# LinjianMa/pairwise-perturbation

Hardware: AMD Instinct MI355X
Metric: ALS sweeps/sec (exact dimension-tree sweep, CP order-4 s=200 R=10) (higher is better)
Workload: dtype f32

## Files before the change

pairwise-perturbation_amd/csrc/engine.cpp:

```cpp
#include "engine.h"
#include "assignment.h"
#include "run_report.h"

#include <algorithm>
#include <cmath>
#include <cstdio>
#include <cstdlib>
#include <cstring>
#include <fstream>
#include <iostream>
#include <limits>
#include <stdexcept>

namespace ppals {

int tensor_create(Ops &ops, Comm &comm, int order, const int64_t *glens, int dtype,
                  TensorDesc *out, std::string *err) {
  if (order < 2 || order > MAX_ORDER) {
    *err = "tensor order must be in [2, 8]";
    return -1;
  }
  if (!ops.supports_storage(dtype))
    throw Unsupported(dtype == BF16 ? "ppals: this back end cannot store a bf16 tensor"
                                    : "ppals: this back end cannot store this tensor type");
// ... 817 lines not shown
    ops_.zero(gradW_[i], n);
    maxs_ = std::max(maxs_, V_.glens[i]);
    maxblk_ = std::max(maxblk_, block_rows(V_.glens[i], P_));
  }
  const size_t sys_n = multi_ ? (size_t)tab_.sq[K_] : (size_t)R_ * R_;
  G_ = DeviceBuffer(ops_, sizeof(double) * N_ * sys_n);
  S_ = DeviceBuffer(ops_, sizeof(double) * sys_n);
  Sinv_ = DeviceBuffer(ops_, sizeof(double) * sys_n);
  gradsq_ = DeviceBuffer(ops_, sizeof(double) * MAX_ORDER * K_);
  scal_ = DeviceBuffer(ops_, sizeof(double) * 4 * MAX_ORDER);
  ops_.zero(gradsq_.as<double>(), sizeof(double) * MAX_ORDER * K_);
  if (dist_) {
    size_t n = sizeof(double) * (size_t)maxblk_ * P_ * R_;
    sendbuf_ = DeviceBuffer(ops_, n);
    recvbuf_ = DeviceBuffer(ops_, sizeof(double) * (size_t)maxblk_ * R_);
    gatherbuf_ = DeviceBuffer(ops_, n);
    ops_.zero(sendbuf_.as<double>(), n);
    ops_.zero(gatherbuf_.as<double>(), n);
  }
  if (const char *e = std::getenv("PPALS_COMM_SMALL_BYTES")) small_msg_bytes_ = std::atoll(e);
  if (const char *e = std::getenv("PPALS_TEST_BLOCKED_UPDATE")) test_blocks_ = std::atoi(e);
  if (N_ < 3) schedule_ = 0;
  if (const char *e = std::getenv("PPALS_PLACE_TUNE")) ms_tune_enabled_ = std::atoi(e) != 0;
  if (const char *e = std::getenv("PPALS_PACK_LAYOUT")) pack_mode_ = std::atoi(e) >= 0 && std::atoi(e) <= 2 ? std::atoi(e) : -1;
  if (N_ >= 3) {
    ms_set_roots(ms_choose_roots());
    ms_scales_ = DeviceBuffer(ops_, sizeof(double) * 32);
  }
  if (V_.generation) tensor_gen_ = *V_.generation;
  {
    Layout nat;
    nat.ptr = V_.data;
    for (int m = 0; m < N_; m++) nat.order.push_back(m);
    lay_.push_back(std::move(nat));
  }
  size_t xmax = 0;
  const bool place = schedule_ == 1 && N_ >= 3 && ms_tune_enabled_ && ms_X_slack() > 0;
  if (place) {
    for (int r = 0; r < N_; r++) {
      if (ms_set_excluded(r, ms_k_, ms_excl_)) continue;
      xmax = std::max(xmax, ms_X_bytes(r, ms_k_));
    }
    const size_t avail = ops_.mem_available();
    const double tensor_bytes = (double)V_.nloc * dtype_size(V_.dtype);
    if (avail == (size_t)-1 || (double)avail > 2.0 * tensor_bytes + 6.0 * (double)(xmax + ms_X_slack()) + 8e9)
      ms_X_alt_ = DeviceBuffer::try_alloc(ops_, xmax + ms_X_slack());
// ... 1134 lines not shown
    ms_start_step(r);
    return;
  }
  const void *src = pl.lay->ptr;
  const int64_t L = pl.Lc, J = pl.J, T = pl.T;
  ms_X_.modes = pl.kept;
  std::vector<FactorRef> f;
  unsigned mask = 0;
  for (int m : pl.set) {
    f.push_back(fref(m, W_.data()));
    mask |= 1u << m;
  }
  ms_X_.dt = work_dt(V_.dtype);
  ms_X_.contracted = mask;
  if ((size_t)L * T * R_ * dtype_size(ms_X_.dt) != xbytes)
    throw std::runtime_error("ppals: internal error (first-level intermediate size)");
  PackedSrc pk_store;
  const PackedSrc *pk = pl.Lc > 1 ? packed_for(pl, pk_store) : nullptr;
  auto launch_scan = [&](int blk, int64_t off, int nt) {
    ms_X_.buf = ms_X_override_ ? (char *)ms_X_override_
                               : (blk == 1 && ms_X_alt_ ? ms_X_alt_ : ms_X_base_).as<char>() + off;
    ops_.scan_store_mode(nt);
    PackedScope scope(ops_, pk);
    ops_.scan_contract(src, V_.dtype, pl.L, J, T, f.data(), (int)f.size(), R_, ms_X_.buf, ms_X_.dt,
                       L, L * T, pl.pad);
    ops_.scan_store_mode(-1);
  };
  PlaceExplore &ex = ms_place_[first];
  if (slack > 0 && !ms_X_override_ && ex.phase < 0) {
    static const int64_t cand_small[] = {0, 1, 2, 3, 4, 5, 6, 8, 12, 16, 24, 32, 48, 64};
    static const int64_t cand_large[] = {0, 3, 5, 12, 16, 24, 48, 64};
    const double bytes = (double)L * J * T * dtype_size(V_.dtype);
    ex.phase = 3;
    ex.layout = (int)(pl.lay - lay_.data());
    if (bytes >= place_min_bytes() && R_ <= 32 && (double)xbytes >= 0.01 * bytes) {
      const bool large = bytes >= 2e10;
      const int64_t *mb = large ? cand_large : cand_small;
      for (int ci = 0; ci < (large ? 8 : 14); ci++) {
        if ((size_t)(mb[ci] << 20) > slack) break;
        PlaceCand c;
        c.off = mb[ci] << 20;
        ex.cands.push_back(c);
      }
      static const int64_t cand_alt[] = {0, 4, 16, 64};
      for (int ci = 0; ms_X_alt_ && ci < 4; ci++) {
        if ((size_t)(cand_alt[ci] << 20) > slack) break;
        PlaceCand c;
        c.blk = 1;
        c.off = cand_alt[ci] << 20;
        ex.cands.push_back(c);
      }
      ex.phase = 0;
    }
  }
  const int cand = (slack > 0 && !ms_X_override_ && ex.phase >= 0 && ex.phase < 2) ? ms_place_pick(ex) : -1;
  if (cand >= 0) {
    ex.visits++;
    ex.timer_cand = cand;
    ex.timer = ops_.timer_begin();
    launch_scan(ex.cands[cand].blk, ex.cands[cand].off, ex.cands[cand].nt);
    if (ex.timer >= 0) ops_.timer_end(ex.timer);
  } else if (ex.phase == 2 && ex.chosen >= 0 && slack > 0 && !ms_X_override_) {
    launch_scan(ex.cands[ex.chosen].blk, ex.cands[ex.chosen].off, ex.cands[ex.chosen].nt);
  } else {
    launch_scan(0, 0, -1);
  }
  ms_X_.pending = false;
  ms_X_.valid = true;
  if (const char *tr = std::getenv("PPALS_TRACE_STEPS")) {
    if (FILE *f = std::fopen(tr, "a")) {
      const int li = (int)(pl.lay - lay_.data());
      std::fprintf(f, "rank=%d root=%d k=%d layout=%s%s L=%lld J=%lld T=%lld\n", rank_, first, k,
                   li == 1 ? "VT" : "V", pl.lay->q > 0 ? "pad" : "", (long long)L, (long long)J,
                   (long long)T);
      std::fclose(f);
    }
  }
}

void CpEngine::ms_mode_update(int i, double lambda, bool last_of_sweep) {
  check_tensor_generation();
  if (kind_[i] == kModeFixed) return;
  if (ms_root_ < 0 || ((i - ms_root_ + N_) % N_) < ms_k_) {
    const int first = ms_next_root(i, ms_k_, ms_excl_);
    if (first < 0) throw std::runtime_error("ppals: no root set without the excluded modes");
    ms_start_step(first);
  }
  int pos = -1;
  for (size_t q = 0; q < ms_order_.size(); q++)
    if (ms_order_[q] == i) pos = (int)q;
  const int leaf = ms_leaf_[pos];
  const bool free_i = kind_[i] == kModeFree;
  if (!multi_ && free_i) ops_.arm_gram_system(G_.as<double>(), N_, i, R_, lambda, S_.as<double>(), Sinv_.as<double>());
  ms_compute(leaf);
  ms_norm_fused_ = false;
  if (last_of_sweep && !multi_ && free_i && !skips_normalize() && (!dist_ || (i != 0 && (int64_t)sizeof(double) * V_.glens[i] * R_ <= small_msg_bytes_))) {
    int64_t rows[MAX_ORDER];
    for (int q = 0; q < N_; q++) rows[q] = V_.glens[q];
    if (ops_.arm_normalize(W_.data(), rows, N_, R_, G_.as<double>(), i, nullptr)) {
      unsigned masks[32] = {0}, fresh = 0;
      const unsigned active = ms_collect_scales(masks, &fresh, leaf);
      ms_norm_fused_ = ops_.arm_normalize(W_.data(), rows, N_, R_, G_.as<double>(), i, nullptr,
                                          ms_scales_.as<double>(), masks, active, fresh);
    }
  }
  mode_update(i, (const double *)ms_nodes_[leaf].t.buf, ext(i), lambda, false, 1.0);
  ms_nodes_[leaf].t.valid = false;
  for (auto &nd : ms_nodes_)
    if (nd.t.contracted & (1u << i)) nd.t.valid = false;
}

void CpEngine::ms_contract(const RTensor &src, int mode, RTensor &dst, DeviceBuffer &own, const double *in_scale) {
  int64_t L = 1, T = 1;
  bool before = true;
  dst.modes.clear();
  for (int m : src.modes) {
    if (m == mode) {
      before = false;
      continue;
    }
    (before ? L : T) *= ext(m);
    dst.modes.push_back(m);
  }
  dst.dt = F64;
  dst.contracted = src.contracted | (1u << mode);
  own.reserve(ops_, sizeof(double) * (size_t)L * T * R_);
  dst.buf = own.get();
  FactorRef f = fref(mode, W_.data());
// ... 15 lines not shown
  auto storage_pos = [&](int mode) {
    for (size_t k = 0; k < src->modes.size(); k++)
      if (src->modes[k] == mode) return (int)k;
    return -1;
  };
  std::sort(sib.begin(), sib.end(), [&](int a, int b) { return storage_pos(a) > storage_pos(b); });
  if (n.tmp.size() + 1 < sib.size()) {
    n.tmp.resize(sib.size() - 1);
    n.tmp_own.resize(sib.size() - 1);
  }
  const RTensor *cur = src;
  for (size_t k = 0; k < sib.size(); k++) {
    const bool last = k + 1 == sib.size();
    RTensor &dst = last ? n.t : n.tmp[k];
    ms_contract(*cur, sib[k], dst, last ? n.own : n.tmp_own[k], k == 0 ? ms_scale_of(*src) : nullptr);
    cur = &dst;
  }
  if (sib.empty()) throw std::runtime_error("ppals: empty sibling set in the multi-sweep tree");
  n.t.pending = false;
  n.t.valid = true;
}

void CpEngine::sweep_msdt(double lambda) {
  for (int i = 0; i < N_; i++) ms_mode_update(i, lambda, i == N_ - 1);
  if (!ms_norm_fused_ && !skips_normalize()) normalize();
  ms_norm_fused_ = false;
  grad_from_sweep_ = true;
}

void CpEngine::sweep_dt(double lambda) {
  if (schedule_ == 1) {
    sweep_msdt(lambda);
    return;
  }
  for (auto &n : nodes_) n.valid = false;
  bool norm_fused = false;
  for (int i = 0; i < N_; i++) {
    if (kind_[i] == kModeFixed) continue;
    compute_node(leaf_[i]);
    const Node &lf = nodes_[leaf_[i]];
    if (i == N_ - 1 && !dist_ && kind_[i] == kModeFree && !skips_normalize()) {
      int64_t rows[MAX_ORDER];
      for (int q = 0; q < N_; q++) rows[q] = V_.glens[q];
      norm_fused = ops_.arm_normalize(W_.data(), rows, N_, R_, G_.as<double>(), i, nullptr);
    }
    mode_update(i, lf.buf.as<double>(), ext(i), lambda, false, 1.0);
  }
// ... 1470 lines not shown
```

pairwise-perturbation_amd/csrc/engine.h:

```cpp
#pragma once
#include <cstdint>
#include <cstdlib>
#include <functional>
#include <map>
#include <string>
#include <vector>

#include "device_buffer.h"
#include "ops.h"

namespace ppals {

struct TensorDesc {
  int order = 0;
  int64_t glens[MAX_ORDER];
  int64_t llens[MAX_ORDER];
  int64_t row0 = 0;
  int dtype = F32;
  void *data = nullptr;
  int64_t nloc = 0;
  uint64_t *generation = nullptr;
  uint64_t *prep_epoch = nullptr;
};

// ... 252 lines not shown
    std::vector<RTensor> tmp;
    DeviceBuffer own;
    std::vector<DeviceBuffer> tmp_own;
  };
  void ms_build_tree(int lo, int hi, int parent);
  void ms_start_step(int root);
  void ms_compute(int idx);
  void ms_contract(const RTensor &src, int mode, RTensor &dst, DeviceBuffer &own, const double *in_scale);
  void sweep_msdt(double lambda);
  void ms_invalidate() { ms_root_ = -1; }
  int schedule_ = 1;
  int ms_root_ = -1;
  int ms_k_ = 1;
  int test_blocks_ = 0;
  DeviceBuffer test_blkbuf_;
  unsigned ms_excl_ = 0;
  bool ms_set_excluded(int first, int k, unsigned excl) const;
  int ms_next_root(int i, int k, unsigned excl) const;
  double ms_schedule_cost(int k, unsigned excl) const;
  int ms_choose_roots();
  void ms_set_roots(int k);
  void ms_mode_update(int i, double lambda, bool last_of_sweep = false);
  bool ms_norm_fused_ = false;
  unsigned ms_collect_scales(unsigned *masks, unsigned *fresh, int skip_node);
  RTensor ms_X_;
  struct PlaceCand {
    int blk = 0;
    int64_t off = 0;
    int nt = -1;
    double best = 1e300;
    int samples = 0;
  };
  struct PlaceExplore {
    int phase = -1;
    size_t next = 0;
    int timer = -1;
    int timer_cand = -1;
    int chosen = -1;
    int layout = 0;
    double worst = 0;
    int visits = 0;
    bool gated = false;
    std::vector<PlaceCand> cands;
  };
  static constexpr int kPlaceGateSamples = 8;
  static constexpr double kPlaceGateSpread = 0.04;
// ... 163 lines not shown
```

pairwise-perturbation_amd/csrc/hip_ops.hip:

```cpp
#include <dlfcn.h>
#include <hip/hip_runtime.h>
#include <chrono>

#include <algorithm>
#include <cstdio>
#include <cstdlib>
#include <stdexcept>
#include <string>
#include <map>
#include <type_traits>
#include <vector>

#include "hip_ops.h"
#include "roctx_ranges.h"
#include "preload_policy.h"
#include "kernels_scan.hip.h"
#include "kernels_pack.hip.h"
#include "kernels_small.hip.h"
#include "kernels_nn.hip.h"
#include "kernels_polar.hip.h"
#include "kernels_shape.hip.h"
#include "kernels_holdout.hip.h"
#include "kernels_corcondia.hip.h"
#include "kernels_fms.hip.h"
// ... 187 lines not shown
    HIP_CHECK(hipFuncSetAttribute((const void *)k_polar_factor, hipFuncAttributeMaxDynamicSharedMemorySize,
                                  96 * 1024));
    HIP_CHECK(hipFuncSetAttribute((const void *)k_shape_columns, hipFuncAttributeMaxDynamicSharedMemorySize,
                                  (int)kShapeLdsBytes));
    HIP_CHECK(hipFuncSetAttribute((const void *)k_p2_polar, hipFuncAttributeMaxDynamicSharedMemorySize, 96 * 1024));
    const void *p2_wide[] = {(const void *)k_p2_project<float, 4>, (const void *)k_p2_project<double, 4>};
    for (const void *k : p2_wide)
      HIP_CHECK(hipFuncSetAttribute(k, hipFuncAttributeMaxDynamicSharedMemorySize, (int)p2_project_lds(64)));
  }
  ~HipOps() override {
    hipSetDevice(dev_);
    hipStreamSynchronize(st_);
    if (st2_) hipStreamSynchronize(st2_);
    for (auto &ev : events_) {
      hipEventDestroy(ev.a);
      hipEventDestroy(ev.b);
    }
    for (auto &t : timers_) {
      hipEventDestroy(t.a);
      hipEventDestroy(t.b);
    }
    if (ws_mttv_) hipFree(ws_mttv_);
    if (ws_pack_) hipFree(ws_pack_);
    if (pack_stats_) hipFree(pack_stats_);
    if (ws_mv_) hipFree(ws_mv_);
    if (ws_hist_) hipFree(ws_hist_);
    if (ws_slab_) hipFree(ws_slab_);
    if (ws_krp_) hipFree(ws_krp_);
    if (ws_part_) hipFree(ws_part_);
    if (ws_small_) hipFree(ws_small_);
    if (ws_big_) hipFree(ws_big_);
    if (ws_big2_) hipFree(ws_big2_);
    if (ws_eig_) hipFree(ws_eig_);
    if (ws_orth_) hipFree(ws_orth_);
    if (ws_pow_) hipFree(ws_pow_);
    if (ws_cold_) hipFree(ws_cold_);
    if (ws_cold2_) hipFree(ws_cold2_);
    if (ws_cholm_) hipFree(ws_cholm_);
    if (ws_gsfb_) hipFree(ws_gsfb_);
    if (ws_jac_) hipFree(ws_jac_);
    if (eig_host_) hipHostFree(eig_host_);
    if (ws_part2_) hipFree(ws_part2_);
    for (auto &kv : eig_state_) {
      if (kv.second.Q) hipFree(kv.second.Q);
      if (kv.second.Qn) hipFree(kv.second.Qn);
      free_lazy(kv.second);
// ... 1501 lines not shown
    if (pad.ld && (L % pad.ld || pad.ld % VEC || pad.valid > pad.ld || pad.valid <= 0 || L == 1))
      throw std::runtime_error("ppals: scan_contract padded rows inconsistent");
    const bool aligned_base = (((uintptr_t)V) & 15) == 0;
    const bool wide_ok = sizeof(TV) == 4 && wide_enabled_ && L > 1 && aligned_base && (L % 4 == 0) &&
                         L >= 4 && (double)L * J * T >= 1.0e6 && 16.0 * (double)L * 4.0 < 2.0e9 &&
                         ((double)J / 16.0 + 1.0) * 8.0 * 1024.0 < 2.0e9;
    int col_step = 64;
    for (int col0 = 0; col0 < R; col0 += col_step) {
      if (wide_ok && R - col0 > 64) {
        col_step = std::min(128, R - col0);
        if constexpr (sizeof(TV) == 4)
          scan_wide((const float *)V, L, J, T, a, col0, col_step, out, out_tstride, out_rstride, out32, pad);
        continue;
      }
      col_step = 64;
      const int ncols = std::min(64, R - col0);
      const int NT = ncols <= 16 ? 1 : (ncols <= 32 ? 2 : (ncols <= 48 ? 3 : 4));
      const int64_t nblk64 = (J + 4 * VEC - 1) / (4 * VEC);
      if (nblk64 > 0x7fffffff) throw std::runtime_error("ppals: contraction extent too large");
      const int nblk = (int)nblk64;
      const size_t pack_bytes = (size_t)nblk * NT * 4 * 16 * VEC * sizeof(TV);
      TV *P = (TV *)ensure(ws_pack_, ws_pack_sz_, pack_bytes);
      const bool prefix = (L == 1);
      hipLaunchKernelGGL(k_krp_pack<TV>, dim3(grid_for((int64_t)nblk * NT * 64 * VEC, 256)),
                         dim3(256), 0, st_, P, nblk, NT, prefix ? 1 : 0, a, J, col0, ncols);
      HIP_CHECK(hipGetLastError());
      double *o = out32 ? (double *)((float *)out + (int64_t)col0 * out_rstride)
                        : out + (int64_t)col0 * out_rstride;
      const double bytes = (double)L * (double)J * (double)T * sizeof(TV) +
                           (double)L * (double)T * ncols * (out32 ? 4.0 : 8.0);
      if (prefix) {
        const int64_t M = J, K = T;
        const bool al = aligned_base && (M % VEC == 0);
        const int64_t ncolgrp = (K + 63) / 64;
        int want = 1;
        const int target = ncu_ * 4;
        if (ncolgrp < target) want = (int)std::min<int64_t>((target + ncolgrp - 1) / ncolgrp,
                                                            std::max(1, nblk / 64));
        const KSplit ks = k_split(nblk, want);
        const int nsplit = ks.nsplit, per = (int)ks.per;
        double *dst = o;
        int dst32 = out32;
        int64_t dst_ks = out_tstride, dst_ns = out_rstride, dst_ss = 0;
        if (nsplit > 1) {
          dst32 = 0;
          dst = (double *)ensure(ws_slab_, ws_slab_sz_, sizeof(double) * nsplit * ncols * K);
          dst_ks = 1;
          dst_ns = K;
          dst_ss = (int64_t)ncols * K;
// ... 529 lines not shown
                              double *dW, int64_t ldd, double ratio, double *S, double *Sinv) override {
    const size_t lds = sizeof(double) * (32 + 2 * (size_t)R * R + 2 * (size_t)R * (R + 1) + 64) + sizeof(int) * 64;
    const size_t stage = 2 * sizeof(double) * (size_t)rows * R;
    if (R > 64 || force_jacobi_ || norm_armed_ || lds + stage > 150 * 1024 || blk * P != rows ||
        blk > 0x7fffffff) {
      route("%s", "update_blocked.unpack");
      Ops::cp_mode_update_blocked(Gall, N, mode, R, lambda, Mblk, blk, P, scratch, W, ldw, grad, ldg, rows,
                                  gradsq, Winit, ldi, dW, ldd, ratio, S, Sinv);
      return;
    }
    update_mblk_ = (int)blk;
    route("%s", "update_blocked.direct");
    cp_mode_update(Gall, N, mode, R, lambda, Mblk, rows, W, ldw, grad, ldg, rows, gradsq, Winit, ldi, dW,
                   ldd, ratio, S, Sinv, nullptr);
    update_mblk_ = 0;
  }
  int update_mblk_ = 0;
  static constexpr int64_t kUpdateRowParallelFrom = 6144;
  void cp_mode_update(double *Gall, int N, int mode, int R, double lambda, const double *M,
                      int64_t ldm, double *W, int64_t ldw, double *grad, int64_t ldg, int64_t rows,
                      double *gradsq, const double *Winit, int64_t ldi, double *dW, int64_t ldd,
                      double ratio, double *S, double *Sinv, double *dwsq) override {
    RoctxRange roctx_("K4-K6 mode update");
    if (R > 64) {
      route("%s", "update.unfused why=R");
      Ops::cp_mode_update(Gall, N, mode, R, lambda, M, ldm, W, ldw, grad, ldg, rows, gradsq, Winit,
                          ldi, dW, ldd, ratio, S, Sinv, dwsq);
      return;
    }
    if (force_jacobi_) {
      route("%s", "update.unfused why=jacobi");
      Ops::cp_mode_update(Gall, N, mode, R, lambda, M, ldm, W, ldw, grad, ldg, rows, gradsq, Winit,
                          ldi, dW, ldd, ratio, S, Sinv, dwsq);
      return;
    }
    if (!Winit) dwsq = nullptr;
    size_t lds = sizeof(double) * (32 + 2 * (size_t)R * R + 2 * (size_t)R * (R + 1) + 64) +
                 sizeof(int) * 64;
    const size_t stage = 2 * sizeof(double) * (size_t)rows * R;
    if (lds + stage > 150 * 1024 && (int64_t)rows * R > kUpdateRowParallelFrom && !norm_armed_ && !update_mblk_) {
      route("%s", "update.unfused why=rows");
      Ops::cp_mode_update(Gall, N, mode, R, lambda, M, ldm, W, ldw, grad, ldg, rows, gradsq, Winit, ldi, dW,
                          ldd, ratio, S, Sinv, dwsq);
      return;
    }
    const int presolved = (sys_ready_ && sys_.Gall == Gall && sys_.mode == mode && sys_.S == S &&
                           sys_.Sinv == Sinv && S && sys_.lambda == lambda) ? 1 : 0;
    sys_ready_ = false;
    sys_armed_ = false;
    NormArgs nrm;
    if (norm_armed_) {
      if (!(norm_.on && norm_mode_ == mode && norm_G_ == Gall && ldw == rows))
        throw std::logic_error("ppals: armed Normalize does not match the mode update that followed");
      nrm = norm_;
      nrm.scales = small(MAX_ORDER);
      norm_armed_ = false;
    }
    if (lds + stage <= 150 * 1024) {
      route("update.staged presolved=%d norm=%d mblk=%d dwsq=%d", presolved, nrm.on ? 1 : 0, update_mblk_ ? 1 : 0,
            dwsq ? 1 : 0);
      hipLaunchKernelGGL((k_cp_mode_update<true, true>), dim3(1), dim3(1024), lds + stage, st_, Gall, N, mode,
                         R, lambda, M, ldm, W, ldw, grad, ldg, rows, gradsq, Winit, ldi, dW, ldd, ratio, S,
                         Sinv, dwsq, presolved, nrm, update_mblk_);
    } else {
      if (update_mblk_) throw std::logic_error("ppals: blocked mode update needs the staged launch");
      route("update.unstaged presolved=%d", presolved);
      hipLaunchKernelGGL((k_cp_mode_update<false, false>), dim3(1), dim3(1024), lds, st_, Gall, N, mode,
                         R, lambda, M, ldm, W, ldw, grad, ldg, rows, gradsq, Winit, ldi, dW, ldd, ratio,
                         S, Sinv, dwsq, presolved);
    }
    HIP_CHECK(hipGetLastError());
  }
  void cp_mode_update_nn(double *Gall, int N, int mode, int R, double lambda, const double *M, int64_t ldm,
                         double *W, int64_t ldw, double *grad, int64_t ldg, int64_t rows, double *gradsq,
                         double *S) override {
    RoctxRange roctx_("K4-K6 mode update (non-negative)");
    if (R > 64) throw Unsupported("ppals: the non-negative mode update supports R <= 64");
    if (sys_armed_ || sys_ready_ || norm_armed_)
      throw std::logic_error("ppals: armed S / Normalize in front of a non-negative mode update");
    if (rows <= 0) {
      HIP_CHECK(hipMemsetAsync(gradsq, 0, sizeof(double), st_));
      gram(W, rows, ldw, R, Gall + (size_t)mode * R * R);
      return;
    }
    const int64_t nb = (rows + 63) / 64;
    if (nb > (int64_t)1 << 30) throw std::runtime_error("ppals: mode too long for the non-negative update");
// ... 371 lines not shown
    }
    norm_mode_ = mode;
    norm_G_ = Gall;
    (void)small(MAX_ORDER);
    norm_armed_ = true;
    route("%s", "arm_normalize.taken");
    return true;
  }
  void arm_gram_system(const double *Gall, int N, int mode, int R, double lambda, double *S,
                       double *Sinv) override {
    sys_ready_ = false;
    sys_armed_ = false;
    if (force_jacobi_ || R > 32 || !S || !Sinv) return;
    sys_.Gall = Gall;
    sys_.N = N;
    sys_.mode = mode;
    sys_.lambda = lambda;
    sys_.S = S;
    sys_.Sinv = Sinv;
    sys_.force_jacobi = 0;
    sys_R_ = R;
    sys_armed_ = true;
  }
  void pp_correct(const double *M0, int64_t rows, int R, const PPTerm *terms, int nterms,
                  double *M) override {
    RoctxRange roctx_("K9 pp_correct");
    if (nterms > MAX_ORDER) throw std::runtime_error("ppals: too many PP correction terms");
    PPTerms tm;
    tm.n = nterms;
    for (int t = 0; t < nterms; t++) {
      tm.T[t] = terms[t].T;
      tm.dW[t] = terms[t].dW;
      tm.ny[t] = terms[t].ny;
      tm.lddw[t] = terms[t].lddw;
      tm.keep_first[t] = terms[t].keep_first;
    }
    dim3 grid((unsigned)((rows + 15) / 16), (unsigned)R);
    SysArgs sys;
    size_t lds = 0;
    if (sys_armed_ && sys_R_ == R) {
      sys = sys_;
      grid.x += 1;
      lds = sizeof(double) * (2 * (size_t)R * (R + 1) + 64) + sizeof(int) * 64;
    }
    route("pp_correct terms=%d extra=%d", nterms, sys.Gall ? 1 : 0);
    prof_begin(1, 0.0);
// ... 27 lines not shown
      return;
    }
    if (R > 64 || (int64_t)rows * R > kUpdateRowParallelFrom) {
      route("%s", "cp_update.rows");
      const int nb = (int)((rows + 63) / 64);
      double *wcopy = (double *)ensure(ws_big2_, ws_big2_sz_,
                                       sizeof(double) * ((size_t)rows * R + (size_t)nb));
      double *part = wcopy + (size_t)rows * R;
      HIP_CHECK(hipMemcpy2DAsync(wcopy, sizeof(double) * rows, Wold, sizeof(double) * ldw,
                                 sizeof(double) * rows, R, hipMemcpyDeviceToDevice, st_));
      hipLaunchKernelGGL(k_cp_update_big, dim3(nb), dim3(256), 0, st_, M, ldm, wcopy, rows, Wnew, ldn,
                         grad, ldg, rows, R, S, Sinv, part, Winit, ldi, dW, ldd, ratio);
      hipLaunchKernelGGL(k_sum_partials, dim3(1), dim3(1024), 0, st_, part, nb, gradsq);
      HIP_CHECK(hipGetLastError());
      return;
    }
    size_t lds = sizeof(double) * (32 + 2 * (size_t)R * R);
    route("%s", "cp_update.one");
    hipLaunchKernelGGL(k_cp_update, dim3(1), dim3(1024), lds, st_, M, ldm, Wold, ldw, Wnew, ldn,
                       grad, ldg, rows, R, S, Sinv, gradsq, Winit, ldi, dW, ldd, ratio);
    HIP_CHECK(hipGetLastError());
  }
  void normalize(double *const *W, const int64_t *rows, int N, int R, double *Gall) override {
    double *scales = small(MAX_ORDER);
    route("%s", "normalize.grid");
    hipLaunchKernelGGL(k_norm_scales, dim3(1), dim3(1024), 0, st_, Gall, N, R, scales);
    HIP_CHECK(hipGetLastError());
    PtrsN w;
    int64_t mx = 1;
    for (int i = 0; i < N; i++) {
      w.p[i] = W[i];
      w.n[i] = rows[i] * R;
      mx = std::max(mx, w.n[i]);
    }
    hipLaunchKernelGGL(k_scale_factors, dim3(grid_for(mx, 256, 64), N), dim3(256), 0, st_, w, N,
                       scales);
    HIP_CHECK(hipGetLastError());
  }
  void normalize_ms(double *const *W, const int64_t *rows, int N, int R, double *Gall,
                    double *ms_dst, const unsigned *masks, unsigned active, unsigned fresh,
                    double *wsq) override {
    RoctxRange roctx_("K7 normalize");
    int64_t tot = 0;
    for (int i = 0; i < N; i++) tot += rows[i] * R;
    if (tot > 65536) {
      Ops::normalize_ms(W, rows, N, R, Gall, ms_dst, masks, active, fresh, wsq);
      return;
    }
    PtrsN w;
    for (int i = 0; i < N; i++) {
      w.p[i] = W[i];
      w.n[i] = rows[i] * R;
    }
    ScaleMasks sm;
    for (int k = 0; k < 32; k++) sm.m[k] = masks ? masks[k] : 0u;
    route("%s", "normalize.fused");
    hipLaunchKernelGGL(k_normalize_fused, dim3(1), dim3(1024), 0, st_, Gall, N, R, w,
                       small(MAX_ORDER), active ? ms_dst : nullptr, sm, active, fresh, wsq);
    HIP_CHECK(hipGetLastError());
  }
  void diff_norms(double *const *A, double *const *B, const int64_t *n, int N, int store_diff,
                  double *const *D, int update_prev, double *out) override {
    PtrsN a;
    for (int i = 0; i < N; i++) {
      a.p[i] = A[i];
// ... 1531 lines not shown
  static constexpr double kNtMinBytes = 192.0 * 1048576.0;
  bool nt_store(int nsplit, double result_bytes) const {
    return nsplit == 1 && (scan_nt_mode_ < 0 ? result_bytes >= kNtMinBytes : scan_nt_mode_ == 1);
  }
  static int occupancy(int &cached, const void *kernel, int block, size_t lds, int fallback) {
    if (cached == 0) {
      int nb = 0;
      const hipError_t e = hipOccupancyMaxActiveBlocksPerMultiprocessor(&nb, kernel, block, lds);
      if (e != hipSuccess) (void)hipGetLastError();
      cached = (e == hipSuccess && nb > 0) ? nb : fallback;
    }
    return cached;
  }

  int dev_ = 0, ncu_ = 256, force_jacobi_ = 0, persist_mult_ = 40;
  int eig_debug_ = 0;
  SysArgs sys_;
  int sys_R_ = 0;
  bool sys_armed_ = false, sys_ready_ = false;
  NormArgs norm_;
  int norm_mode_ = -1;
  const double *norm_G_ = nullptr;
  bool norm_armed_ = false;
  bool eig_frob_once_ = false;
  void *ws_jac_ = nullptr;
  size_t ws_jac_sz_ = 0;
  int sym_lds_min_ = 768;
  int eig_defer_ok_ = 1;
  bool handover_ok_ = true;
  unsigned long long *handover_ = nullptr;
  unsigned long long handover_seq_ = 0;
  int eig_defer_fail_ = 0;
  int eig_defer_count_ = 0;
  int eig_cold_ = 1;
  void *ws_cold_ = nullptr;
  size_t ws_cold_sz_ = 0;
  double eig_sigma_scale_ = 0;
  int force_eiginv_ = 0;
  int eig_fast_ = 1;
  std::map<int, EigState> eig_state_;
  int eig_next_base_ = 0;
  void *eig_host_ = nullptr;
  void *ws_eig_ = nullptr, *ws_orth_ = nullptr, *ws_pow_ = nullptr, *ws_part2_ = nullptr;
  size_t ws_eig_sz_ = 0, ws_orth_sz_ = 0, ws_pow_sz_ = 0, ws_part2_sz_ = 0;
  hipStream_t st_ = nullptr;
  hipStream_t st2_ = nullptr;
// ... 22 lines not shown
```

pairwise-perturbation_amd/csrc/kernels_scan.hip.h:

```cpp
#pragma once
#include <hip/hip_runtime.h>
#include <stdint.h>

#include "ops.h"

namespace ppals {

typedef float f32x4 __attribute__((ext_vector_type(4)));
typedef double f64x4 __attribute__((ext_vector_type(4)));
typedef double f64x2 __attribute__((ext_vector_type(2)));

template <typename TV>
struct ScanTraits;
template <>
struct ScanTraits<float> {
  static constexpr int VEC = 4;
  typedef f32x4 vec;
  typedef f32x4 acc;
  static constexpr bool NEEDS_FLUSH = true;
  __device__ static inline acc mfma(float a, float b, acc c) {
    return __builtin_amdgcn_mfma_f32_16x16x4f32(a, b, c, 0, 0, 0);
  }
  __device__ static inline int row(int lane, int reg) { return (lane >> 4) * 4 + reg; }
};
// ... 1508 lines not shown
__global__ void k_rank_pack(const double *__restrict__ P, int64_t K, int R, int RB, int nkb,
                            double *__restrict__ Ppk) {
  const int64_t total = (int64_t)nkb * RB * 64;
  for (int64_t e = (int64_t)blockIdx.x * blockDim.x + threadIdx.x; e < total;
       e += (int64_t)gridDim.x * blockDim.x) {
    const int i = (int)(e & 15), g = (int)((e >> 4) & 3);
    const int64_t t = e >> 6;
    const int rb = (int)(t % RB);
    const int64_t kb = t / RB;
    const int64_t k = kb * 16 + i;
    const int r = 4 * rb + g;
    Ppk[e] = (k < K && r < R) ? P[k + K * (int64_t)r] : 0.0;
  }
}

struct KrpArgs {
  const double *ptr[MAX_ORDER];
  int64_t rows[MAX_ORDER];
  int64_t ld[MAX_ORDER];
  int nf;
};

template <typename TV>
__global__ void k_krp_pack(TV *__restrict__ P, int nblk, int NT, int prefix_layout, KrpArgs a,
                           int64_t J, int col0, int ncols) {
  constexpr int VEC = ScanTraits<TV>::VEC;
  const int64_t total = (int64_t)nblk * NT * 4 * 16 * VEC;
  for (int64_t e = (int64_t)blockIdx.x * blockDim.x + threadIdx.x; e < total;
       e += (int64_t)gridDim.x * blockDim.x) {
    int64_t t = e;
    const int u = (int)(t % VEC);
    t /= VEC;
    const int n = (int)(t % 16);
    t /= 16;
    const int g = (int)(t % 4);
    t /= 4;
    const int nt = (int)(t % NT);
    const int64_t blk = t / NT;
    const int64_t j = blk * 4 * VEC + (prefix_layout ? VEC * g + u : 4 * u + g);
    const int c = 16 * nt + n;
    double v = 0.0;
    if (j < J && c < ncols) {
      v = 1.0;
      int64_t rem = j;
      for (int f = 0; f < a.nf; f++) {
        const int64_t jf = rem % a.rows[f];
        rem /= a.rows[f];
        v *= a.ptr[f][jf + a.ld[f] * (col0 + c)];
      }
    }
    P[e] = (TV)v;
  }
}

__global__ void k_slab_reduce(const double *__restrict__ slab, int nsplit, int64_t split_stride,
                              int64_t M, int ncols, double *__restrict__ out, int64_t out_mstride,
                              int64_t out_rstride, int out32, int64_t row_ld, int64_t row_valid,
                              int64_t slab_batch_stride = 0, int64_t out_batch_stride = 0) {
  slab += (int64_t)blockIdx.y * slab_batch_stride;
  const int64_t obatch = (int64_t)blockIdx.y * out_batch_stride;
  const int64_t total = M * ncols;
  for (int64_t e = (int64_t)blockIdx.x * blockDim.x + threadIdx.x; e < total;
       e += (int64_t)gridDim.x * blockDim.x) {
    const int64_t m = e % M;
    const int64_t n = e / M;
    const ScanRowMap rm = scan_row_map<1>(m, M, row_ld, row_valid);
    if (rm.nvalid == 0) continue;
    double s = 0;
    for (int sp = 0; sp < nsplit; sp++) s += slab[sp * split_stride + e];
    scan_store(out, obatch + rm.mo * out_mstride + out_rstride * n, s, out32);
  }
}

}
```

pairwise-perturbation_amd/csrc/kernels_small.hip.h:

```cpp
#pragma once
#include <hip/hip_runtime.h>
#include <stdint.h>

#include "kernels_scan.hip.h"

namespace ppals {

typedef double f64x4 __attribute__((ext_vector_type(4)));


__host__ __device__ inline uint64_t splitmix64(uint64_t x) {
  x += 0x9E3779B97F4A7C15ull;
  x = (x ^ (x >> 30)) * 0xBF58476D1CE4E5B9ull;
  x = (x ^ (x >> 27)) * 0x94D049BB133111EBull;
  return x ^ (x >> 31);
}
__host__ __device__ inline double u01(uint64_t seed, uint64_t idx) {
  uint64_t h = splitmix64(splitmix64(seed) ^ idx);
  return (double)(h >> 11) * (1.0 / 9007199254740992.0);
}

__device__ inline double wave_sum(double v) {
#pragma unroll
  for (int off = 32; off > 0; off >>= 1) v += __shfl_down(v, off, 64);
// ... 1278 lines not shown

struct PtrsN {
  double *p[MAX_ORDER];
  double *q[MAX_ORDER];
  double *d[MAX_ORDER];
  int64_t n[MAX_ORDER];
};
struct NormArgs {
  int on = 0;
  PtrsN w;
  double *scales = nullptr;
  double *wsq = nullptr;
  double *ms_dst = nullptr;
  ScaleMasks masks;
  unsigned active = 0, fresh = 0;
};
#ifdef PPALS_UPDATE_STAMPS
__device__ unsigned long long g_update_stamps[16];
#define PPALS_STAMP(i) \
  if (threadIdx.x == 0) g_update_stamps[i] = __builtin_amdgcn_s_memrealtime()
#else
#define PPALS_STAMP(i)
#endif
template <bool STAGE, bool MF, bool NORM>
__device__ __forceinline__ void cp_mode_update_body(
    double *__restrict__ Gall, int N, int mode, int R, double lambda, const double *__restrict__ M,
    int64_t ldm, double *W, int64_t ldw, double *__restrict__ grad, int64_t ldg, int64_t rows,
    double *__restrict__ gradsq, const double *__restrict__ Winit, int64_t ldi,
    double *__restrict__ dW, int64_t ldd, double ratio, double *__restrict__ S_out,
    double *__restrict__ Sinv_out, double *__restrict__ dwsq, int presolved, const NormArgs &nrm,
    int mblk) {
  extern __shared__ double lds[];
  const int ldA = R + 1;
  double *red = lds;
  double *sS = lds + 32;
  double *sI = sS + R * R;
  double *A = sI + R * R;
  double *Q = A + R * ldA;
  double *cs = Q + R * ldA;
  int *pq = (int *)(cs + 64);
  const int tid = threadIdx.x, lane = tid & 63, wave = tid >> 6;
  double *sM = (double *)(pq + 64);
  double *sW = sM + (STAGE ? rows * R : 0);
  const int64_t total = rows * R;
  const int rows_i = (int)rows, total_i = (int)total;
  PPALS_STAMP(0);

  if (presolved) {
    for (int e = tid; e < R * R; e += blockDim.x) {
      sS[e] = S_out[e];
      sI[e] = Sinv_out[e];
    }
    if (STAGE)
      for (int e = tid; e < total_i; e += (int)blockDim.x) {
// ... 108 lines not shown
      for (int k = 0; k < R; k++) acc += M[i + ldm * k] * sI[k + R * j];
    }
    if (Winit) {
      const double wi = Winit[i + ldi * j];
      const double d = ratio * (acc - wi);
      dW[i + ldd * j] = d;
      dd += d * d;
      if (ratio != 1.0) acc = wi + d;
    }
    W[i + ldw * j] = acc;
    if (STAGE) sW[e] = acc;
  }
  }
  if (dwsq) {
    dd = (STAGE && MF) ? block_sum_lds(dd, red + 16) : block_sum(dd, red);
    if (tid == 0) *dwsq = dd;
  }
  PPALS_STAMP(4);
  if constexpr (STAGE && MF)
    lds_barrier();
  else
    __syncthreads();
  PPALS_STAMP(5);
  double *G = Gall + (int64_t)mode * R * R;
  const int nw = blockDim.x >> 6;
  if constexpr (STAGE && MF) {
    const int g4 = lane >> 4, l16 = lane & 15;
    const int ntg = (R + 15) / 16, ntile = ntg * (ntg + 1) / 2;
    const int cap = (int)((rows * R) / (ntile * 256));
    const int nks = cap < 1 ? 0 : (cap < nw ? cap : nw);
    if (nks > 0) {
      const int ksteps = (rows_i + 3) / 4, spw = (ksteps + nks - 1) / nks;
      if (wave < nks) {
        const int s0 = wave * spw, s1 = (s0 + spw < ksteps) ? s0 + spw : ksteps;
        int t = 0;
        for (int tp = 0; tp < ntg; tp++)
          for (int tq = tp; tq < ntg; tq++, t++) {
            const int ca = 16 * tp + l16, cb = 16 * tq + l16;
            f64x4 acc = {0.0, 0.0, 0.0, 0.0}, acc2 = {0.0, 0.0, 0.0, 0.0};
            for (int ks = s0; ks < s1; ks += 2) {
              const int k = 4 * ks + g4, k2 = k + 4;
              const bool kin = k < rows_i, kin2 = (ks + 1 < s1) && k2 < rows_i;
              const double a = (kin && ca < R) ? sW[k + rows_i * ca] : 0.0;
              const double b = (kin && cb < R) ? sW[k + rows_i * cb] : 0.0;
              const double a2 = (kin2 && ca < R) ? sW[k2 + rows_i * ca] : 0.0;
              const double b2 = (kin2 && cb < R) ? sW[k2 + rows_i * cb] : 0.0;
// ... 90 lines not shown
        if (i == mode) {
          for (int e = tid; e < total_i; e += (int)blockDim.x)
            W[(e % rows_i) + ldw * (e / rows_i)] = f * sW[e];
        } else {
          for (int64_t e = tid; e < nrm.w.n[i]; e += blockDim.x) pw[e] = f * pw[e];
        }
      }
      if (nrm.ms_dst && tid < 32 && ((nrm.active >> tid) & 1u)) {
        double v = ((nrm.fresh >> tid) & 1u) ? 1.0 : nrm.ms_dst[tid];
        for (int m = 0; m < MAX_ORDER; m++)
          if (nrm.masks.m[tid] & (1u << m)) v *= nr[MAX_ORDER + m];
        nrm.ms_dst[tid] = v;
      }
    }
  }
}
template <bool STAGE, bool MF = false>
__global__ __launch_bounds__(1024) void k_cp_mode_update(
    double *__restrict__ Gall, int N, int mode, int R, double lambda, const double *__restrict__ M,
    int64_t ldm, double *W, int64_t ldw, double *__restrict__ grad, int64_t ldg, int64_t rows,
    double *__restrict__ gradsq, const double *__restrict__ Winit, int64_t ldi,
    double *__restrict__ dW, int64_t ldd, double ratio, double *__restrict__ S_out,
    double *__restrict__ Sinv_out, double *__restrict__ dwsq, int presolved = 0,
    NormArgs nrm = NormArgs(), int mblk = 0) {
  cp_mode_update_body<STAGE, MF, true>(Gall, N, mode, R, lambda, M, ldm, W, ldw, grad, ldg, rows, gradsq, Winit,
                                 ldi, dW, ldd, ratio, S_out, Sinv_out, dwsq, presolved, nrm, mblk);
}
template <bool STAGE, bool MF = false>
__global__ __launch_bounds__(1024) void k_cp_mode_update_batched(
    double *__restrict__ Gall, int N, int mode, int R, double lambda, const double *__restrict__ M,
    int64_t ldm, double *W, int64_t ldw, double *__restrict__ grad, int64_t ldg, int64_t rows,
    double *__restrict__ gradsq, double *__restrict__ S_out, double *__restrict__ Sinv_out) {
  const int64_t b = blockIdx.x;
  const int64_t c0 = b * R, rr = (int64_t)R * R;
  cp_mode_update_body<STAGE, MF, false>(Gall + b * N * rr, N, mode, R, lambda, M + c0 * ldm, ldm, W + c0 * ldw, ldw,
                                 grad + c0 * ldg, ldg, rows, gradsq + b, nullptr, 0, nullptr, 0, 1.0,
                                 S_out ? S_out + b * rr : nullptr, Sinv_out ? Sinv_out + b * rr : nullptr,
                                 nullptr, 0, NormArgs(), 0);
}

template <bool STAGE, bool MF = false>
__global__ __launch_bounds__(1024) void k_cp_mode_update_ragged(
    double *__restrict__ Gall, int N, int mode, StartTable t, double lambda, const double *__restrict__ M,
    int64_t ldm, double *W, int64_t ldw, double *__restrict__ grad, int64_t ldg, int64_t rows,
    double *__restrict__ gradsq, double *__restrict__ S_out, double *__restrict__ Sinv_out) {
  const int b = blockIdx.x;
  const int64_t c0 = t.col[b], so = t.sq[b];
  cp_mode_update_body<STAGE, MF, false>(Gall + N * so, N, mode, t.col[b + 1] - t.col[b], lambda, M + c0 * ldm, ldm,
                                 W + c0 * ldw, ldw, grad + c0 * ldg, ldg, rows, gradsq + b, nullptr, 0, nullptr,
// ... 278 lines not shown
```

pairwise-perturbation_amd/csrc/ops.h:

```cpp
#pragma once
#include <cmath>
#include <cstddef>
#include <cstdint>
#include <limits>
#include <string>
#include <vector>

#include "bf16.h"
#include "device_view.h"
#include "pack_codec.h"
#include "preload_policy.h"

namespace ppals {

enum DType { F32 = 0, F64 = 1, BF16 = 3 };
inline size_t dtype_size(int dt) { return dt == F32 ? 4 : (dt == BF16 ? 2 : 8); }
inline int work_dt(int storage) { return storage == BF16 ? F32 : storage; }

struct RowPad {
  int64_t ld = 0, valid = 0;
};

struct PackedSrc {
  const void *data = nullptr;
// ... 1001 lines not shown
    std::vector<double> q(nq), p(np), as((size_t)A, 0.0), bs((size_t)B, 0.0);
    d2h(raw.data(), V, raw.size());
    d2h(q.data(), Q, sizeof(double) * nq);
    d2h(p.data(), P, sizeof(double) * np);
    if (!first) d2h(as.data(), asq, sizeof(double) * as.size());
    for (int64_t b = 0; b < B; b++) {
      const int64_t pb = (b % mp.pL) + mp.pLK * (b / mp.pL);
      for (int64_t a = 0; a < A; a++) {
        double v = 0;
        for (int k = 0; k < K; k++) v += q[(size_t)(a + mp.ldq * k)] * p[(size_t)(pb + mp.pL * k)];
        const size_t e = (size_t)(mp.roff + ra[(size_t)a] + rb[(size_t)b]);
        const double x = dt == F32 ? (double)((const float *)raw.data())[e] : ((const double *)raw.data())[e];
        const double d = x - v;
        as[(size_t)a] += d * d;
        bs[(size_t)b] += d * d;
      }
    }
    h2d(asq, as.data(), sizeof(double) * as.size());
    h2d(bsq, bs.data(), sizeof(double) * bs.size());
  }
  virtual void scan_profile_slot(int ) {}
  virtual void arm_gram_system(const double * , int , int , int ,
                               double , double * , double * ) {}
  virtual bool arm_normalize(double *const * , const int64_t * , int , int ,
                             double * , int , double * ,
                             double *  = nullptr, const unsigned *  = nullptr,
                             unsigned  = 0, unsigned  = 0) {
    return false;
  }
  virtual void normalize(double *const *W, const int64_t *rows, int N, int R, double *Gall) = 0;
  virtual void diff_norms(double *const *A, double *const *B, const int64_t *n, int N,
                          int store_diff, double *const *D, int update_prev, double *out) = 0;
  virtual void pack_blocks(const double *nat, int64_t rows, int64_t ld, int R, int64_t blk, int P,
                           double *blocked) = 0;
  virtual void unpack_blocks(const double *blocked, int64_t rows, int64_t ld, int R, int64_t blk,
                             int P, double *nat) = 0;

  virtual void unfold_gram(const void *X, int dt, int64_t L, int64_t J, int64_t T, double *G) = 0;
  virtual void top_eigvecs(double *G, int64_t J, int rank, double *U) = 0;
  virtual void top_eigvecs_warm(double *G, int64_t J, int rank, double *U, int ) {
    top_eigvecs(G, J, rank, U);
  }
  virtual void eig_lazy(int , bool ) {}
  virtual void eig_defer(int , bool ) {}
  virtual double *eig_gram(int , int64_t ) { return nullptr; }
  virtual bool eig_deferred(int ) { return false; }
// ... 48 lines not shown
```

Baseline: 720.0.

## Fuse next scan's KRP factor packing into the staged mode-update kernel

When a mode update is the last leaf of a root step and the next scan will contract only this freshly updated factor, the staged mode-update kernel now writes the packed KRP operand (f32) from its LDS copy of W. The following scan_contract detects the matching prepacked buffer and skips its separate k_krp_pack launch. The goal is to remove one kernel launch and a reread of the factor per step. In exchange the single-block update kernel does extra serial packing work, and correctness depends on pointer/shape matching and on invalidation in normalize paths.

Result: slower. 687.9 (-4.5%).

```diff
diff --git a/pairwise-perturbation_amd/csrc/engine.cpp b/pairwise-perturbation_amd/csrc/engine.cpp
--- a/pairwise-perturbation_amd/csrc/engine.cpp
+++ b/pairwise-perturbation_amd/csrc/engine.cpp
@@ -863,6 +863,7 @@
   if (const char *e = std::getenv("PPALS_TEST_BLOCKED_UPDATE")) test_blocks_ = std::atoi(e);
   if (N_ < 3) schedule_ = 0;
   if (const char *e = std::getenv("PPALS_PLACE_TUNE")) ms_tune_enabled_ = std::atoi(e) != 0;
+  if (const char *e = std::getenv("PPALS_STEP_FUSE")) step_fuse_ = std::atoi(e) != 0;
   if (const char *e = std::getenv("PPALS_PACK_LAYOUT")) pack_mode_ = std::atoi(e) >= 0 && std::atoi(e) <= 2 ? std::atoi(e) : -1;
   if (N_ >= 3) {
     ms_set_roots(ms_choose_roots());
@@ -2043,8 +2044,10 @@
                                : (blk == 1 && ms_X_alt_ ? ms_X_alt_ : ms_X_base_).as<char>() + off;
     ops_.scan_store_mode(nt);
     PackedScope scope(ops_, pk);
+    const int64_t by_update = ops_.krp_pack_fused();
     ops_.scan_contract(src, V_.dtype, pl.L, J, T, f.data(), (int)f.size(), R_, ms_X_.buf, ms_X_.dt,
                        L, L * T, pl.pad);
+    ms_scan_prepacked_ = ops_.krp_pack_fused() > by_update;
     ops_.scan_store_mode(-1);
   };
   PlaceExplore &ex = ms_place_[first];
@@ -2091,9 +2094,9 @@
   if (const char *tr = std::getenv("PPALS_TRACE_STEPS")) {
     if (FILE *f = std::fopen(tr, "a")) {
       const int li = (int)(pl.lay - lay_.data());
-      std::fprintf(f, "rank=%d root=%d k=%d layout=%s%s L=%lld J=%lld T=%lld\n", rank_, first, k,
+      std::fprintf(f, "rank=%d root=%d k=%d layout=%s%s L=%lld J=%lld T=%lld krp=%s\n", rank_, first, k,
                    li == 1 ? "VT" : "V", pl.lay->q > 0 ? "pad" : "", (long long)L, (long long)J,
-                   (long long)T);
+                   (long long)T, ms_scan_prepacked_ ? "update" : "launch");
       std::fclose(f);
     }
   }
@@ -2125,6 +2128,12 @@
                                           ms_scales_.as<double>(), masks, active, fresh);
     }
   }
+  if (step_fuse_ && ms_in_sweep_ && !last_of_sweep && !multi_ && !dist_ && free_i && ms_k_ == 1 &&
+      pos + 1 == (int)ms_order_.size() && !ms_X_override_ && test_blocks_ <= 1 &&
+      ms_next_root((i + 1) % N_, 1, ms_excl_) == i) {
+    ScanPlan next;
+    if (plan_scan(i, 1, false, next)) ops_.arm_krp_pack(V_.dtype, next.L == 1 ? 1 : 0);
+  }
   mode_update(i, (const double *)ms_nodes_[leaf].t.buf, ext(i), lambda, false, 1.0);
   ms_nodes_[leaf].t.valid = false;
   for (auto &nd : ms_nodes_)
@@ -2186,7 +2195,15 @@
 }
 
 void CpEngine::sweep_msdt(double lambda) {
-  for (int i = 0; i < N_; i++) ms_mode_update(i, lambda, i == N_ - 1);
+  struct InSweep {
+    bool &f;
+    explicit InSweep(bool &b) : f(b) { f = true; }
+    ~InSweep() { f = false; }
+  };
+  {
+    InSweep in(ms_in_sweep_);
+    for (int i = 0; i < N_; i++) ms_mode_update(i, lambda, i == N_ - 1);
+  }
   if (!ms_norm_fused_ && !skips_normalize()) normalize();
   ms_norm_fused_ = false;
   grad_from_sweep_ = true;
diff --git a/pairwise-perturbation_amd/csrc/engine.h b/pairwise-perturbation_amd/csrc/engine.h
--- a/pairwise-perturbation_amd/csrc/engine.h
+++ b/pairwise-perturbation_amd/csrc/engine.h
@@ -298,6 +298,9 @@
   void ms_set_roots(int k);
   void ms_mode_update(int i, double lambda, bool last_of_sweep = false);
   bool ms_norm_fused_ = false;
+  bool step_fuse_ = true;
+  bool ms_in_sweep_ = false;
+  bool ms_scan_prepacked_ = false;
   unsigned ms_collect_scales(unsigned *masks, unsigned *fresh, int skip_node);
   RTensor ms_X_;
   struct PlaceCand {
diff --git a/pairwise-perturbation_amd/csrc/hip_ops.hip b/pairwise-perturbation_amd/csrc/hip_ops.hip
--- a/pairwise-perturbation_amd/csrc/hip_ops.hip
+++ b/pairwise-perturbation_amd/csrc/hip_ops.hip
@@ -233,6 +233,7 @@
     }
     if (ws_mttv_) hipFree(ws_mttv_);
     if (ws_pack_) hipFree(ws_pack_);
+    if (ws_prepack_) hipFree(ws_prepack_);
     if (pack_stats_) hipFree(pack_stats_);
     if (ws_mv_) hipFree(ws_mv_);
     if (ws_hist_) hipFree(ws_hist_);
@@ -1780,9 +1781,22 @@
       const size_t pack_bytes = (size_t)nblk * NT * 4 * 16 * VEC * sizeof(TV);
       TV *P = (TV *)ensure(ws_pack_, ws_pack_sz_, pack_bytes);
       const bool prefix = (L == 1);
-      hipLaunchKernelGGL(k_krp_pack<TV>, dim3(grid_for((int64_t)nblk * NT * 64 * VEC, 256)),
-                         dim3(256), 0, st_, P, nblk, NT, prefix ? 1 : 0, a, J, col0, ncols);
-      HIP_CHECK(hipGetLastError());
+      bool packed = false;
+      if constexpr (std::is_same<TV, float>::value) {
+        const Prepacked &pp = prepacked_;
+        packed = pp.P && nf == 1 && a.ptr[0] == pp.W && a.ld[0] == pp.ld && a.rows[0] == pp.rows && col0 == 0 &&
+                 ncols == pp.R && R == pp.R && (prefix ? 1 : 0) == pp.prefix && pp.P == (float *)ws_prepack_;
+        if (packed) P = pp.P;
+      }
+      prepacked_ = Prepacked();
+      if (packed) {
+        krp_pack_fused_++;
+        route("%s", "krp_pack.by_update");
+      } else {
+        hipLaunchKernelGGL(k_krp_pack<TV>, dim3(grid_for((int64_t)nblk * NT * 64 * VEC, 256)),
+                           dim3(256), 0, st_, P, nblk, NT, prefix ? 1 : 0, a, J, col0, ncols);
+        HIP_CHECK(hipGetLastError());
+      }
       double *o = out32 ? (double *)((float *)out + (int64_t)col0 * out_rstride)
                         : out + (int64_t)col0 * out_rstride;
       const double bytes = (double)L * (double)J * (double)T * sizeof(TV) +
@@ -2358,6 +2372,9 @@
                       double *gradsq, const double *Winit, int64_t ldi, double *dW, int64_t ldd,
                       double ratio, double *S, double *Sinv, double *dwsq) override {
     RoctxRange roctx_("K4-K6 mode update");
+    const bool want_pack = pack_armed_;
+    pack_armed_ = false;
+    prepacked_ = Prepacked();
     if (R > 64) {
       route("%s", "update.unfused why=R");
       Ops::cp_mode_update(Gall, N, mode, R, lambda, M, ldm, W, ldw, grad, ldg, rows, gradsq, Winit,
@@ -2392,12 +2409,26 @@
       nrm.scales = small(MAX_ORDER);
       norm_armed_ = false;
     }
+    KrpPackArgs pk;
+    if (want_pack && pack_armed_dt_ == F32 && rows > 0 && lds + stage <= 150 * 1024 && !nrm.on) {
+      constexpr int VEC = ScanTraits<float>::VEC;
+      pk.NT = R <= 16 ? 1 : (R <= 32 ? 2 : (R <= 48 ? 3 : 4));
+      pk.nblk = (int)((rows + 4 * VEC - 1) / (4 * VEC));
+      pk.prefix = pack_armed_prefix_;
+      pk.P = (float *)ensure(ws_prepack_, ws_prepack_sz_, (size_t)pk.nblk * pk.NT * 4 * 16 * VEC * sizeof(float));
+      prepacked_.W = W;
+      prepacked_.ld = ldw;
+      prepacked_.rows = rows;
+      prepacked_.R = R;
+      prepacked_.prefix = pk.prefix;
+      prepacked_.P = pk.P;
+    }
     if (lds + stage <= 150 * 1024) {
-      route("update.staged presolved=%d norm=%d mblk=%d dwsq=%d", presolved, nrm.on ? 1 : 0, update_mblk_ ? 1 : 0,
-            dwsq ? 1 : 0);
+      route("update.staged presolved=%d norm=%d mblk=%d dwsq=%d pack=%d", presolved, nrm.on ? 1 : 0,
+            update_mblk_ ? 1 : 0, dwsq ? 1 : 0, pk.P ? 1 : 0);
       hipLaunchKernelGGL((k_cp_mode_update<true, true>), dim3(1), dim3(1024), lds + stage, st_, Gall, N, mode,
                          R, lambda, M, ldm, W, ldw, grad, ldg, rows, gradsq, Winit, ldi, dW, ldd, ratio, S,
-                         Sinv, dwsq, presolved, nrm, update_mblk_);
+                         Sinv, dwsq, presolved, nrm, update_mblk_, pk);
     } else {
       if (update_mblk_) throw std::logic_error("ppals: blocked mode update needs the staged launch");
       route("update.unstaged presolved=%d", presolved);
@@ -2815,6 +2846,12 @@
     sys_R_ = R;
     sys_armed_ = true;
   }
+  void arm_krp_pack(int dt, int prefix) override {
+    pack_armed_ = true;
+    pack_armed_dt_ = dt;
+    pack_armed_prefix_ = prefix ? 1 : 0;
+  }
+  int64_t krp_pack_fused() override { return krp_pack_fused_; }
   void pp_correct(const double *M0, int64_t rows, int R, const PPTerm *terms, int nterms,
                   double *M) override {
     RoctxRange roctx_("K9 pp_correct");
@@ -2888,6 +2925,7 @@
     HIP_CHECK(hipGetLastError());
   }
   void normalize(double *const *W, const int64_t *rows, int N, int R, double *Gall) override {
+    prepacked_ = Prepacked();
     double *scales = small(MAX_ORDER);
     route("%s", "normalize.grid");
     hipLaunchKernelGGL(k_norm_scales, dim3(1), dim3(1024), 0, st_, Gall, N, R, scales);
@@ -2907,6 +2945,7 @@
                     double *ms_dst, const unsigned *masks, unsigned active, unsigned fresh,
                     double *wsq) override {
     RoctxRange roctx_("K7 normalize");
+    prepacked_ = Prepacked();
     int64_t tot = 0;
     for (int i = 0; i < N; i++) tot += rows[i] * R;
     if (tot > 65536) {
@@ -4484,6 +4523,18 @@
   int norm_mode_ = -1;
   const double *norm_G_ = nullptr;
   bool norm_armed_ = false;
+  struct Prepacked {
+    const double *W = nullptr;
+    int64_t ld = 0, rows = 0;
+    int R = 0, prefix = 0;
+    float *P = nullptr;
+  };
+  Prepacked prepacked_;
+  bool pack_armed_ = false;
+  int pack_armed_dt_ = 0, pack_armed_prefix_ = 0;
+  int64_t krp_pack_fused_ = 0;
+  void *ws_prepack_ = nullptr;
+  size_t ws_prepack_sz_ = 0;
   bool eig_frob_once_ = false;
   void *ws_jac_ = nullptr;
   size_t ws_jac_sz_ = 0;
diff --git a/pairwise-perturbation_amd/csrc/kernels_scan.hip.h b/pairwise-perturbation_amd/csrc/kernels_scan.hip.h
--- a/pairwise-perturbation_amd/csrc/kernels_scan.hip.h
+++ b/pairwise-perturbation_amd/csrc/kernels_scan.hip.h
@@ -1554,35 +1554,41 @@
 };
 
 template <typename TV>
+__device__ __forceinline__ TV krp_pack_entry(int64_t e, int NT, int prefix_layout, const KrpArgs &a, int64_t J,
+                                             int col0, int ncols) {
+  constexpr int VEC = ScanTraits<TV>::VEC;
+  int64_t t = e;
+  const int u = (int)(t % VEC);
+  t /= VEC;
+  const int n = (int)(t % 16);
+  t /= 16;
+  const int g = (int)(t % 4);
+  t /= 4;
+  const int nt = (int)(t % NT);
+  const int64_t blk = t / NT;
+  const int64_t j = blk * 4 * VEC + (prefix_layout ? VEC * g + u : 4 * u + g);
+  const int c = 16 * nt + n;
+  double v = 0.0;
+  if (j < J && c < ncols) {
+    v = 1.0;
+    int64_t rem = j;
+    for (int f = 0; f < a.nf; f++) {
+      const int64_t jf = rem % a.rows[f];
+      rem /= a.rows[f];
+      v *= a.ptr[f][jf + a.ld[f] * (col0 + c)];
+    }
+  }
+  return (TV)v;
+}
+
+template <typename TV>
 __global__ void k_krp_pack(TV *__restrict__ P, int nblk, int NT, int prefix_layout, KrpArgs a,
                            int64_t J, int col0, int ncols) {
   constexpr int VEC = ScanTraits<TV>::VEC;
   const int64_t total = (int64_t)nblk * NT * 4 * 16 * VEC;
   for (int64_t e = (int64_t)blockIdx.x * blockDim.x + threadIdx.x; e < total;
-       e += (int64_t)gridDim.x * blockDim.x) {
-    int64_t t = e;
-    const int u = (int)(t % VEC);
-    t /= VEC;
-    const int n = (int)(t % 16);
-    t /= 16;
-    const int g = (int)(t % 4);
-    t /= 4;
-    const int nt = (int)(t % NT);
-    const int64_t blk = t / NT;
-    const int64_t j = blk * 4 * VEC + (prefix_layout ? VEC * g + u : 4 * u + g);
-    const int c = 16 * nt + n;
-    double v = 0.0;
-    if (j < J && c < ncols) {
-      v = 1.0;
-      int64_t rem = j;
-      for (int f = 0; f < a.nf; f++) {
-        const int64_t jf = rem % a.rows[f];
-        rem /= a.rows[f];
-        v *= a.ptr[f][jf + a.ld[f] * (col0 + c)];
-      }
-    }
-    P[e] = (TV)v;
-  }
+       e += (int64_t)gridDim.x * blockDim.x)
+    P[e] = krp_pack_entry<TV>(e, NT, prefix_layout, a, J, col0, ncols);
 }
 
 __global__ void k_slab_reduce(const double *__restrict__ slab, int nsplit, int64_t split_stride,
diff --git a/pairwise-perturbation_amd/csrc/kernels_small.hip.h b/pairwise-perturbation_amd/csrc/kernels_small.hip.h
--- a/pairwise-perturbation_amd/csrc/kernels_small.hip.h
+++ b/pairwise-perturbation_amd/csrc/kernels_small.hip.h
@@ -1324,6 +1324,10 @@
 #else
 #define PPALS_STAMP(i)
 #endif
+struct KrpPackArgs {
+  float *P = nullptr;
+  int nblk = 0, NT = 0, prefix = 0;
+};
 template <bool STAGE, bool MF, bool NORM>
 __device__ __forceinline__ void cp_mode_update_body(
     double *__restrict__ Gall, int N, int mode, int R, double lambda, const double *__restrict__ M,
@@ -1331,7 +1335,7 @@
     double *__restrict__ gradsq, const double *__restrict__ Winit, int64_t ldi,
     double *__restrict__ dW, int64_t ldd, double ratio, double *__restrict__ S_out,
     double *__restrict__ Sinv_out, double *__restrict__ dwsq, int presolved, const NormArgs &nrm,
-    int mblk) {
+    int mblk, const KrpPackArgs &pk = KrpPackArgs()) {
   extern __shared__ double lds[];
   const int ldA = R + 1;
   double *red = lds;
@@ -1486,6 +1490,18 @@
   else
     __syncthreads();
   PPALS_STAMP(5);
+  if constexpr (STAGE) {
+    if (pk.P) {
+      KrpArgs a;
+      a.ptr[0] = sW;
+      a.rows[0] = rows;
+      a.ld[0] = rows;
+      a.nf = 1;
+      const int npk = pk.nblk * pk.NT * (4 * 16 * ScanTraits<float>::VEC);
+      for (int e = tid; e < npk; e += (int)blockDim.x)
+        pk.P[e] = krp_pack_entry<float>(e, pk.NT, pk.prefix, a, rows, 0, R);
+    }
+  }
   double *G = Gall + (int64_t)mode * R * R;
   const int nw = blockDim.x >> 6;
   if constexpr (STAGE && MF) {
@@ -1622,9 +1638,9 @@
     double *__restrict__ gradsq, const double *__restrict__ Winit, int64_t ldi,
     double *__restrict__ dW, int64_t ldd, double ratio, double *__restrict__ S_out,
     double *__restrict__ Sinv_out, double *__restrict__ dwsq, int presolved = 0,
-    NormArgs nrm = NormArgs(), int mblk = 0) {
+    NormArgs nrm = NormArgs(), int mblk = 0, KrpPackArgs pk = KrpPackArgs()) {
   cp_mode_update_body<STAGE, MF, true>(Gall, N, mode, R, lambda, M, ldm, W, ldw, grad, ldg, rows, gradsq, Winit,
-                                 ldi, dW, ldd, ratio, S_out, Sinv_out, dwsq, presolved, nrm, mblk);
+                                 ldi, dW, ldd, ratio, S_out, Sinv_out, dwsq, presolved, nrm, mblk, pk);
 }
 template <bool STAGE, bool MF = false>
 __global__ __launch_bounds__(1024) void k_cp_mode_update_batched(
diff --git a/pairwise-perturbation_amd/csrc/ops.h b/pairwise-perturbation_amd/csrc/ops.h
--- a/pairwise-perturbation_amd/csrc/ops.h
+++ b/pairwise-perturbation_amd/csrc/ops.h
@@ -1047,6 +1047,8 @@
   virtual void scan_profile_slot(int ) {}
   virtual void arm_gram_system(const double * , int , int , int ,
                                double , double * , double * ) {}
+  virtual void arm_krp_pack(int , int ) {}
+  virtual int64_t krp_pack_fused() { return 0; }
   virtual bool arm_normalize(double *const * , const int64_t * , int , int ,
                              double * , int , double * ,
                              double *  = nullptr, const unsigned *  = nullptr,
```
